# felipefelixarias/a2cat-vn-pytorch

Measured on AMD Instinct MI355X. Metric: env-steps/sec (whole node), 4096 parallel cached-THOR envs at 1/2/4/8 GPUs, higher is better.
Workload: dtype u8; 1 GPU; cached-THOR VectorEnv.step, 20 synthetic 24x24 scenes (626 MB frame cache, HBM-resident), 4096 envs/GPU, 84x84x3 frames, uniform random actions, auto-reset, TimeLimit 900; envs_per_gpu=4096, scenes=20, parallelism=dp1 (independent env shards, replicated scene cache)

## Files before the change

a2cat-vn-pytorch_amd/csrc/vn_env.hip:

```cpp
#include <hip/hip_runtime.h>

#include <algorithm>
#include <cstdlib>
#include <cstring>
#include <mutex>
#include <new>
#include <vector>

#include "vn_common.h"

namespace vn {

static thread_local std::string g_last_error;
void set_error(const std::string& msg) { g_last_error = msg; }
int fail(int code, const std::string& msg) {
  set_error(msg);
  return code;
}
int hip_fail(hipError_t e, const char* what) {
  set_error(std::string(what) + ": " + hipGetErrorString(e));
  return VN_EHIP;
}
const std::string& last_error() { return g_last_error; }

struct SceneDev {
  int64_t row_base;
  int64_t spd_off;
  int64_t cnt_off;
  int64_t comp_base;
  int32_t graph_off;
  int32_t n;
  int32_t maxd;
  int32_t cur_oi;
  int32_t cur_mode;
  float r_goal, r_step, r_coll;
  int32_t terminal_obs;
};

enum { ST_SCENE = 0, ST_STATE, ST_GOAL, ST_OBS, ST_ELAPSED, ST_EPISODE, ST_SCHED, ST_COUNT };

struct EnvArgs {
  const SceneDev* scenes;
  const int32_t* graph;
  const int32_t* spd;
  const uint8_t* arena;
  int64_t frame_bytes;
  int32_t* st;
  float* ep_ret;
  const int32_t* env_scene;
  const int32_t* tasks;
  const int32_t* sched;
  const int32_t* cur_order;
  const int32_t* cur_count;
  uint32_t* flags;
  int n_tasks, sched_len, max_steps, autoreset, n_envs;
  int cur_mode;
  uint32_t k0, k1;
  const int32_t* actions;
  const int32_t* mask;
  uint8_t* obs;
  uint8_t* goal_out;
  float* reward;
  uint8_t* done;
  int32_t* state_out;
  float* info_ret;
  int32_t* info_len;
  int32_t* info_term;
  uint8_t* info_trunc;
  int32_t* info_img_row;
  int32_t* info_goal_row;
  const float* pol_out;
  int pol_A;
  uint32_t pk0, pk1;
  const int64_t* pctr_dev;
  uint64_t pctr;
  int32_t* act_out;
  int64_t* prev_action;
  float* prev_reward;
  float* prev_mask;
  float* lra_next;
  float* mask_next;
  float* stats_env;
  const float* head_w;
  const float* head_b;
  const float* head_x;
  float* head_out;
  uint64_t* rec_addr;
  int32_t* rec_row;
  int reuse;
};

enum { MODE_STEP = 0, MODE_RESET = 1, MODE_OBSERVE = 2, MODE_STEP_HEADS = 3 };
constexpr int kEnvsPerBlock = 4;
constexpr int kStartRounds = 16;

__device__ __forceinline__ int uni(int v) { return __builtin_amdgcn_readfirstlane(v); }

__device__ void reset_env(const EnvArgs& a, int e, int lane, int& sc, int& s, int& g) {
  const int n_envs = a.n_envs;
  const int k = a.st[ST_EPISODE * n_envs + e];
  const int sp = a.st[ST_SCHED * n_envs + e];
  if (a.sched_len > 0 && sp < a.sched_len) {
    sc = a.env_scene[e];
    const int n = a.scenes[sc].n;
    s = a.sched[((int64_t)e * a.sched_len + sp) * 2 + 0];
    g = a.sched[((int64_t)e * a.sched_len + sp) * 2 + 1];
    if ((unsigned)s >= (unsigned)n || (unsigned)g >= (unsigned)n) {
      if (lane == 0) atomicOr(a.flags, (uint32_t)VN_FLAG_BAD_SCHEDULE);
      s = min(max(s, 0), n - 1);
      g = min(max(g, 0), n - 1);
    }
    if (lane == 0) a.st[ST_SCHED * n_envs + e] = sp + 1;
    return;
  }
  const u32x4 rg = philox4x32_10(u32x4{(uint32_t)e, (uint32_t)k, 0u, STREAM_GOAL}, a.k0, a.k1);
  if (a.n_tasks > 0) {
    const int t = (int)uniform_below(rg.x, (uint32_t)a.n_tasks);
    sc = a.tasks[2 * t];
    g = a.tasks[2 * t + 1];
    if (g < 0) g = (int)uniform_below(rg.y, (uint32_t)a.scenes[sc].n);
  } else {
    sc = a.env_scene[e];
    g = (int)uniform_below(rg.x, (uint32_t)a.scenes[sc].n);
  }
  const SceneDev S = a.scenes[sc];
  const int32_t* spd = a.spd + S.spd_off;
  s = -1;
  if (a.cur_mode > 0 && S.cur_mode > 0) {
    const int oi = S.cur_oi;
    const int32_t* cnt = a.cur_count + S.cnt_off + (int64_t)g * (S.maxd + 2);
    const int lo = cnt[1], hi = cnt[oi + 1], n = S.n;
    const u32x4 r = philox4x32_10(u32x4{(uint32_t)e, (uint32_t)k, 0u, STREAM_START}, a.k0, a.k1);
    const bool use_far = (S.cur_mode == 2 && r.y >= 3865470566u && hi < n) || hi <= lo;
    const int b0 = use_far ? hi : lo, b1 = use_far ? n : hi;
    if (b1 > b0) s = a.cur_order[S.spd_off + (int64_t)g * n + b0 + (int)uniform_below(r.x, (uint32_t)(b1 - b0))];
  }
  for (int round = 0; round < kStartRounds && s < 0; ++round) {
    const uint32_t att = (uint32_t)(round * 64 + lane);
    const u32x4 r = philox4x32_10(u32x4{(uint32_t)e, (uint32_t)k, att, STREAM_START}, a.k0, a.k1);
    const int cand = (int)uniform_below(r.x, (uint32_t)S.n);
    const bool ok = spd[(int64_t)cand * S.n + g] > 0;
    const unsigned long long m = __ballot(ok);
    if (m) {
      s = __shfl(cand, __ffsll((long long)m) - 1);
      break;
    }
  }
  if (s < 0) {
    if (lane == 0) atomicOr(a.flags, (uint32_t)VN_FLAG_RESET_EXHAUSTED);
    const u32x4 r = philox4x32_10(u32x4{(uint32_t)e, (uint32_t)k, 0u, STREAM_START}, a.k0, a.k1);
    s = (int)uniform_below(r.x, (uint32_t)S.n);
  }
  s = uni(s);
}

__device__ __forceinline__ void st16_nt(uint4* p, const uint4 v) {
  __builtin_nontemporal_store(v.x, &p->x);
  __builtin_nontemporal_store(v.y, &p->y);
  __builtin_nontemporal_store(v.z, &p->z);
  __builtin_nontemporal_store(v.w, &p->w);
}

template <int VEC>
__device__ __forceinline__ void copy_two_frames(uint8_t* __restrict__ d1, const uint8_t* __restrict__ s1,
                                                uint8_t* __restrict__ d2, const uint8_t* __restrict__ s2,
                                                int64_t bytes, int lane) {
  if constexpr (VEC == 16) {
    constexpr int U = 4;
    const int n = (int)(bytes >> 4);
    const uint4* a = reinterpret_cast<const uint4*>(s1);
    const uint4* b = reinterpret_cast<const uint4*>(s2);
    uint4* x = reinterpret_cast<uint4*>(d1);
    uint4* y = reinterpret_cast<uint4*>(d2);
    int i = lane;
    for (; i + 64 * (U - 1) < n; i += 64 * U) {
      uint4 va[U], vb[U];
#pragma unroll
      for (int u = 0; u < U; ++u) va[u] = a[i + 64 * u];
#pragma unroll
      for (int u = 0; u < U; ++u) vb[u] = b[i + 64 * u];
#pragma unroll
      for (int u = 0; u < U; ++u) st16_nt(x + i + 64 * u, va[u]);
#pragma unroll
      for (int u = 0; u < U; ++u) st16_nt(y + i + 64 * u, vb[u]);
    }
    for (; i < n; i += 64) {
      const uint4 a0 = a[i], b0 = b[i];
      st16_nt(x + i, a0);
      st16_nt(y + i, b0);
    }
  } else if constexpr (VEC == 4) {
    const int n = (int)(bytes >> 2);
    const uint32_t* a = reinterpret_cast<const uint32_t*>(s1);
    const uint32_t* b = reinterpret_cast<const uint32_t*>(s2);
    uint32_t* x = reinterpret_cast<uint32_t*>(d1);
    uint32_t* y = reinterpret_cast<uint32_t*>(d2);
    for (int i = lane; i < n; i += 64) {
      const uint32_t a0 = a[i], b0 = b[i];
      x[i] = a0;
      y[i] = b0;
    }
  } else {
    for (int64_t i = lane; i < bytes; i += 64) {
      d1[i] = s1[i];
      d2[i] = s2[i];
    }
  }
}

template <int VEC>
__device__ __forceinline__ void copy_one_frame(uint8_t* __restrict__ d, const uint8_t* __restrict__ s,
                                               int64_t bytes, int lane) {
  if constexpr (VEC == 16) {
    constexpr int U = 8;
    const int n = (int)(bytes >> 4);
    const uint4* a = reinterpret_cast<const uint4*>(s);
    uint4* x = reinterpret_cast<uint4*>(d);
    int base = 0;
    for (; base + 64 * U <= n; base += 64 * U) {
      const int i = base + lane;
      uint4 v[U];
#pragma unroll
      for (int u = 0; u < U; ++u) v[u] = a[i + 64 * u];
#pragma unroll
      for (int u = 0; u < U; ++u) st16_nt(x + i + 64 * u, v[u]);
    }
    if (base < n) {
      const int i = base + lane;
      uint4 v[U] = {};
#pragma unroll
      for (int u = 0; u < U; ++u)
        if (i + 64 * u < n) v[u] = a[i + 64 * u];
#pragma unroll
      for (int u = 0; u < U; ++u)
        if (i + 64 * u < n) st16_nt(x + i + 64 * u, v[u]);
    }
  } else if constexpr (VEC == 4) {
    const int n = (int)(bytes >> 2);
    const uint32_t* a = reinterpret_cast<const uint32_t*>(s);
    uint32_t* x = reinterpret_cast<uint32_t*>(d);
    for (int i = lane; i < n; i += 64) x[i] = a[i];
  } else {
    for (int64_t i = lane; i < bytes; i += 64) d[i] = s[i];
  }
}

template <int MODE, int VEC>
__global__ __launch_bounds__(256) void env_kernel(EnvArgs a) {
  const int lane = threadIdx.x & 63;
  const int e = uni(blockIdx.x * kEnvsPerBlock + (threadIdx.x >> 6));
  if (e >= a.n_envs) return;
  const int n_envs = a.n_envs;
  int32_t* st = a.st;

  int sc = st[ST_SCENE * n_envs + e];
  int s = st[ST_STATE * n_envs + e];
  int g = st[ST_GOAL * n_envs + e];
  int os = st[ST_OBS * n_envs + e];
  uint64_t rec_a1 = 0, rec_a2 = 0;
  int32_t rec_r1 = -1, rec_r2 = -1;
  if (MODE != MODE_STEP_HEADS && a.reuse) {
    rec_a1 = a.rec_addr[e];
    rec_a2 = a.rec_addr[n_envs + e];
    rec_r1 = a.rec_row[e];
    rec_r2 = a.rec_row[n_envs + e];
  }

  if constexpr (MODE == MODE_STEP || MODE == MODE_STEP_HEADS) {
    int t = st[ST_ELAPSED * n_envs + e];
    const SceneDev S = a.scenes[sc];
    int act;
    if (a.pol_out) {
      float lg[7], p[7], lp[7], H;
      if constexpr (MODE == MODE_STEP_HEADS) {
        const int kl = lane & 31;
        const float* x = a.head_x + (int64_t)e * 512;
        float4 xv[4];
#pragma unroll
        for (int i = 0; i < 4; ++i) xv[i] = *reinterpret_cast<const float4*>(x + 4 * kl + 128 * i);
        float sj[8], bj[8];
#pragma unroll
        for (int j = 0; j < 8; ++j) bj[j] = a.head_b[min(j, a.pol_A)];
#pragma unroll
        for (int j = 0; j < 8; ++j) {
          const float* w = a.head_w + (int64_t)min(j, a.pol_A) * 512;
          float s = 0.0f;
#pragma unroll
          for (int i = 0; i < 4; ++i) {
            const float4 wv = *reinterpret_cast<const float4*>(w + 4 * kl + 128 * i);
            s = fmaf(xv[i].x, wv.x, s);
            s = fmaf(xv[i].y, wv.y, s);
            s = fmaf(xv[i].z, wv.z, s);
            s = fmaf(xv[i].w, wv.w, s);
          }
          sj[j] = s;
        }
#pragma unroll
        for (int j = 0; j < 8; ++j) {
#pragma unroll
          for (int o = 16; o > 0; o >>= 1) sj[j] += __shfl_xor(sj[j], o, 32);
        }
#pragma unroll
        for (int j = 0; j < 8; ++j) {
          if (j <= a.pol_A) {
            const float v = sj[j] + bj[j];
            if (j < a.pol_A) lg[j] = v;
            if (lane == 0) a.head_out[(int64_t)e * 8 + j] = v;
          }
        }
      } else {
        for (int j = 0; j < a.pol_A; ++j) lg[j] = a.pol_out[(int64_t)e * 8 + j];
      }
      const uint64_t ctr = a.pctr + (a.pctr_dev ? (uint64_t)*a.pctr_dev : 0ull);
      act = uni(sample_action(lg, a.pol_A, a.pk0, a.pk1, ctr, (uint32_t)e, p, lp, H));
    } else {
      act = a.actions[e];
    }
    const bool bad = (unsigned)act > 3u;
    int nxt = -1;
    if (!bad) nxt = a.graph[((int64_t)S.graph_off + s) * 4 + act];
    const bool collided = nxt == -1;
    if (!collided) s = nxt;
    const bool terminal = (s == g);
    float r = S.r_step;
    if (terminal) r = S.r_goal;
    if (collided) r = S.r_coll;
    if (!terminal || S.terminal_obs) os = s;
    t += 1;
    const bool limit = a.max_steps > 0 && t >= a.max_steps;
    const bool done = terminal || limit;
    const float ret = a.ep_ret[e] + r;
    const int term_state = os;
    const int ep_len = t;
    float new_ret = ret;
    if (done && a.autoreset) {
      reset_env(a, e, lane, sc, s, g);
      os = s;
      t = 0;
      new_ret = 0.0f;
    }
    if (lane == 0) {
      st[ST_SCENE * n_envs + e] = sc;
      st[ST_STATE * n_envs + e] = s;
      st[ST_GOAL * n_envs + e] = g;
      st[ST_OBS * n_envs + e] = os;
      st[ST_ELAPSED * n_envs + e] = t;
      if (done && a.autoreset) st[ST_EPISODE * n_envs + e] += 1;
      a.ep_ret[e] = new_ret;
      if (bad) atomicOr(a.flags, (uint32_t)VN_FLAG_BAD_ACTION);
      if (a.reward) a.reward[e] = r;
      if (a.done) a.done[e] = done ? 1 : 0;
      if (a.state_out) a.state_out[e] = s;
      if (a.info_ret) a.info_ret[e] = ret;
      if (a.info_len) a.info_len[e] = ep_len;
      if (a.info_term) a.info_term[e] = term_state;
      if (a.info_trunc) a.info_trunc[e] = (limit && !terminal) ? 1 : 0;
      if (a.pol_out) {
        const float m = done ? 0.0f : 1.0f;
        a.act_out[e] = act;
        if (a.prev_action) a.prev_action[e] = act;
        if (a.prev_reward) a.prev_reward[e] = r;
        if (a.prev_mask) a.prev_mask[e] = m;
        if (a.mask_next) a.mask_next[e] = m;
        if (a.lra_next) {
          for (int j = 0; j < a.pol_A; ++j) a.lra_next[(int64_t)e * (a.pol_A + 1) + j] = j == act ? m : 0.0f;
          a.lra_next[(int64_t)e * (a.pol_A + 1) + a.pol_A] = r * m;
        }
        if (a.stats_env && done) {
          a.stats_env[e] += 1.0f;
          a.stats_env[n_envs + e] += ret;
          a.stats_env[2 * (int64_t)n_envs + e] += (float)ep_len;
        }
      }
    }
  } else if constexpr (MODE == MODE_RESET) {
    if (a.mask == nullptr || a.mask[e] != 0) {
      reset_env(a, e, lane, sc, s, g);
      os = s;
      if (lane == 0) {
        st[ST_SCENE * n_envs + e] = sc;
        st[ST_STATE * n_envs + e] = s;
        st[ST_GOAL * n_envs + e] = g;
        st[ST_OBS * n_envs + e] = os;
        st[ST_ELAPSED * n_envs + e] = 0;
        st[ST_EPISODE * n_envs + e] += 1;
        a.ep_ret[e] = 0.0f;
      }
    }
    return;
  } else {
    if (lane == 0 && a.state_out) a.state_out[e] = s;
  }

  const int64_t base = a.scenes[sc].row_base, comp = a.scenes[sc].comp_base;
  const int64_t img_row = base + os, goal_row = comp >= 0 ? comp + os : base + g;
  if (lane == 0) {
    if (a.info_img_row) a.info_img_row[e] = (int32_t)img_row;
    if (a.info_goal_row) a.info_goal_row[e] = (int32_t)goal_row;
  }
  if constexpr (MODE == MODE_STEP_HEADS) return;
  if (a.obs != nullptr && a.goal_out != nullptr) {
    const int64_t F = a.frame_bytes;
    uint8_t* d1 = a.obs + (int64_t)e * F;
    uint8_t* d2 = a.goal_out + (int64_t)e * F;
    const bool keep1 = a.reuse && rec_a1 == (uint64_t)d1 && rec_r1 == (int32_t)img_row;
    const bool keep2 = a.reuse && rec_a2 == (uint64_t)d2 && rec_r2 == (int32_t)goal_row;
    if (!keep1 && !keep2)
      copy_two_frames<VEC>(d1, a.arena + img_row * F, d2, a.arena + goal_row * F, F, lane);
    else if (!keep1)
      copy_one_frame<VEC>(d1, a.arena + img_row * F, F, lane);
    else if (!keep2)
      copy_one_frame<VEC>(d2, a.arena + goal_row * F, F, lane);
    if (lane == 0) {
      a.rec_addr[e] = (uint64_t)d1;
      a.rec_addr[n_envs + e] = (uint64_t)d2;
      a.rec_row[e] = (int32_t)img_row;
      a.rec_row[n_envs + e] = (int32_t)goal_row;
    }
  } else if (a.obs != nullptr || a.goal_out != nullptr) {
    const int64_t F = a.frame_bytes;
    const int k = a.obs ? 0 : 1;
    uint8_t* d = (k == 0 ? a.obs : a.goal_out) + (int64_t)e * F;
    const uint8_t* src = a.arena + (k == 0 ? img_row : goal_row) * F;
    for (int64_t i = lane; i < F; i += 64) d[i] = src[i];
    if (lane == 0) {
      a.rec_addr[k * n_envs + e] = (uint64_t)d;
      a.rec_row[k * n_envs + e] = (int32_t)(k == 0 ? img_row : goal_row);
      if (a.rec_addr[(1 - k) * n_envs + e] == (uint64_t)d) a.rec_addr[(1 - k) * n_envs + e] = 0;
    }
  }
}

__global__ void synth_frames_kernel(uint8_t* arena, int64_t row_base, int n_rows, int64_t frame_bytes,
                                    uint32_t scene_id) {
  const int64_t words = frame_bytes >> 2;
  const int64_t total = words * n_rows;
  uint32_t* dst = reinterpret_cast<uint32_t*>(arena + row_base * frame_bytes);
  for (int64_t i = blockIdx.x * (int64_t)blockDim.x + threadIdx.x; i < total;
       i += (int64_t)gridDim.x * blockDim.x) {
    const int64_t row = i / words, w = i - row * words;
    dst[i] = frame_hash(scene_id, (uint32_t)row, (uint32_t)w);
  }
}

__global__ __launch_bounds__(256) void gather_rows_kernel(const uint8_t* __restrict__ src, int64_t row_bytes,
                                                          const int32_t* __restrict__ rows, int n,
                                                          uint8_t* __restrict__ dst) {
  const int lane = threadIdx.x & 63;
  const int i = uni(blockIdx.x * 4 + (threadIdx.x >> 6));
  if (i >= n) return;
  const uint8_t* s = src + (int64_t)rows[i] * row_bytes;
  uint8_t* d = dst + (int64_t)i * row_bytes;
  if ((row_bytes & 15) == 0) {
    const uint4* a = reinterpret_cast<const uint4*>(s);
    uint4* b = reinterpret_cast<uint4*>(d);
    for (int64_t j = lane; j < (row_bytes >> 4); j += 64) b[j] = a[j];
  } else {
    for (int64_t j = lane; j < row_bytes; j += 64) d[j] = s[j];
  }
}

__global__ void random_actions_kernel(int32_t* actions, int n, uint32_t k0, uint32_t k1, uint64_t step) {
  const int e = blockIdx.x * blockDim.x + threadIdx.x;
  if (e >= n) return;
  const u32x4 r = philox4x32_10(u32x4{(uint32_t)e, (uint32_t)step, (uint32_t)(step >> 32), STREAM_ACTION}, k0, k1);
  actions[e] = (int32_t)(r.x >> 30);
}

}

using namespace vn;

struct vn_ctx {
  int device = 0;
  int n_envs = 0, n_scenes = 0;
  uint64_t seed = 0;
  int64_t frame_bytes = 0, n_rows = 0;
  uint8_t* arena = nullptr;
  int32_t* graph = nullptr;
  int32_t* spd = nullptr;
  SceneDev* scenes = nullptr;
  std::vector<SceneDev> scenes_host;
  int32_t* st = nullptr;
  float* ep_ret = nullptr;
  int32_t* env_scene = nullptr;
  int32_t* tasks = nullptr;
  int n_tasks = 0;
  int32_t* sched = nullptr;
  int sched_len = 0;
  std::vector<int32_t> spd_host;
  int32_t* cur_order = nullptr;
  int32_t* cur_count = nullptr;
  int cur_mode = 0;
  double cur_c = 0.0;
  uint32_t* flags = nullptr;
  int max_steps = 900, autoreset = 1;
  float* info_ret = nullptr;
  int32_t* info_len = nullptr;
  int32_t* info_term = nullptr;
  uint8_t* info_trunc = nullptr;
  int32_t* info_img_row = nullptr;
  int32_t* info_goal_row = nullptr;
  uint64_t* rec_addr = nullptr;
  int32_t* rec_row = nullptr;
  int reuse = 0;
  int reuse_arm = 0;
};

namespace {

struct DeviceGuard {
  int prev = -1;
  explicit DeviceGuard(int d) {
    if (hipGetDevice(&prev) != hipSuccess) prev = -1;
    (void)hipSetDevice(d);
  }
  ~DeviceGuard() {
    if (prev >= 0) (void)hipSetDevice(prev);
  }
};

EnvArgs make_args(vn_ctx* c) {
  EnvArgs a;
  std::memset(&a, 0, sizeof(a));
  a.scenes = c->scenes;
  a.graph = c->graph;
  a.spd = c->spd;
  a.arena = c->arena;
  a.frame_bytes = c->frame_bytes;
  a.st = c->st;
  a.ep_ret = c->ep_ret;
  a.env_scene = c->env_scene;
  a.tasks = c->tasks;
  a.sched = c->sched;
  a.cur_order = c->cur_order;
  a.cur_count = c->cur_count;
  a.cur_mode = c->cur_mode;
  a.flags = c->flags;
  a.n_tasks = c->n_tasks;
  a.sched_len = c->sched_len;
  a.max_steps = c->max_steps;
  a.autoreset = c->autoreset;
  a.n_envs = c->n_envs;
  a.k0 = (uint32_t)c->seed;
  a.k1 = (uint32_t)(c->seed >> 32);
  a.info_ret = c->info_ret;
  a.info_len = c->info_len;
  a.info_term = c->info_term;
  a.info_trunc = c->info_trunc;
  a.info_img_row = c->info_img_row;
  a.info_goal_row = c->info_goal_row;
  a.rec_addr = c->rec_addr;
  a.rec_row = c->rec_row;
  return a;
}

int take_reuse(vn_ctx* c, const uint8_t* obs, const uint8_t* goal, hipStream_t stream) {
  if (!obs || !goal || !c->reuse) return 0;
  if (!c->reuse_arm) return 1;
  hipStreamCaptureStatus cap = hipStreamCaptureStatusNone;
  if (hipStreamIsCapturing(stream, &cap) != hipSuccess) {
    (void)hipGetLastError();
    cap = hipStreamCaptureStatusNone;
  }
  if (cap == hipStreamCaptureStatusNone) c->reuse_arm = 0;
  return 0;
}

template <int MODE>
int launch_env(vn_ctx* c, const EnvArgs& a, hipStream_t stream) {
  const dim3 grid((c->n_envs + kEnvsPerBlock - 1) / kEnvsPerBlock), block(64 * kEnvsPerBlock);
  const int64_t F = c->frame_bytes;
  const bool al16 = (F % 16 == 0) && ((uintptr_t)a.obs % 16 == 0) && ((uintptr_t)a.goal_out % 16 == 0);
  const bool al4 = (F % 4 == 0) && ((uintptr_t)a.obs % 4 == 0) && ((uintptr_t)a.goal_out % 4 == 0);
  if (al16)
    hipLaunchKernelGGL((env_kernel<MODE, 16>), grid, block, 0, stream, a);
  else if (al4)
    hipLaunchKernelGGL((env_kernel<MODE, 4>), grid, block, 0, stream, a);
  else
    hipLaunchKernelGGL((env_kernel<MODE, 1>), grid, block, 0, stream, a);
  VN_HIP(hipGetLastError());
  return VN_OK;
}

void free_ctx(vn_ctx* c) {
  if (!c) return;
  void* ptrs[] = {c->arena, c->graph, c->spd, c->scenes, c->st, c->ep_ret, c->env_scene,
                  c->tasks, c->sched, c->flags, c->cur_order, c->cur_count, c->rec_addr, c->rec_row};
  for (void* p : ptrs)
    if (p) (void)hipFree(p);
  delete c;
}

}

extern "C" {

const char* vn_version(void) { return "vnav 0.1.0 gfx950"; }

int vn_last_error(char* buf, size_t len) {
  if (!buf || len == 0) return VN_EINVAL;
  const std::string& m = vn::last_error();
  const size_t n = std::min(len - 1, m.size());
  std::memcpy(buf, m.data(), n);
  buf[n] = 0;
  return VN_OK;
}

int vn_create(const vn_scene_desc* scenes, int n_scenes, int n_envs, uint64_t seed, int device,
              vn_ctx** out) {
  if (!out) return fail(VN_EINVAL, "vn_create: out is NULL");
  *out = nullptr;
  if (!scenes || n_scenes <= 0) return fail(VN_EINVAL, "vn_create: need at least one scene");
  if (n_envs <= 0) return fail(VN_EINVAL, "vn_create: n_envs must be > 0");
  const int H = scenes[0].height, W = scenes[0].width, C = scenes[0].channels;
  if (H <= 0 || W <= 0 || C <= 0) return fail(VN_EINVAL, "vn_create: bad frame shape");
  const int64_t F = (int64_t)H * W * C;
  int64_t rows = 0, graph_rows = 0, spd_elems = 0;
  std::vector<SceneDev> sh(n_scenes);
  for (int k = 0; k < n_scenes; ++k) {
    const vn_scene_desc& d = scenes[k];
// ... 30 lines not shown
      if (v < -1 || v >= n) return fail(VN_EINVAL, "vn_create: graph entry out of range");
      g32[(int64_t)sh[k].graph_off * 4 + i] = (int32_t)v;
    }
    int32_t mx = 0;
    for (int64_t i = 0; i < n * n; ++i) {
      const int64_t v = d.spd[i];
      spd32[sh[k].spd_off + i] = (int32_t)std::max<int64_t>(std::min<int64_t>(v, INT32_MAX), INT32_MIN);
      mx = std::max(mx, spd32[sh[k].spd_off + i]);
    }
    if (mx > (1 << 20)) return fail(VN_EINVAL, "vn_create: spd values above 2^20");
    sh[k].maxd = mx;
  }
  int64_t cnt_elems = 0;
  for (int k = 0; k < n_scenes; ++k) {
    sh[k].cnt_off = cnt_elems;
    cnt_elems += (int64_t)sh[k].n * (sh[k].maxd + 2);
  }
  DeviceGuard guard(device);
  vn_ctx* c = new (std::nothrow) vn_ctx();
  if (!c) return fail(VN_ENOMEM, "vn_create: host allocation failed");
  c->device = device;
  c->n_envs = n_envs;
  c->n_scenes = n_scenes;
  c->seed = seed;
  c->frame_bytes = F;
  c->n_rows = rows;
  c->scenes_host = sh;
  c->spd_host = spd32;
  auto alloc = [&](void** p, size_t bytes) -> bool {
    return hipMalloc(p, std::max<size_t>(bytes, 16)) == hipSuccess;
  };
  bool ok = alloc((void**)&c->arena, (size_t)(rows * F)) && alloc((void**)&c->graph, g32.size() * 4) &&
            alloc((void**)&c->spd, spd32.size() * 4) && alloc((void**)&c->scenes, sh.size() * sizeof(SceneDev)) &&
            alloc((void**)&c->st, (size_t)ST_COUNT * n_envs * 4) && alloc((void**)&c->ep_ret, (size_t)n_envs * 4) &&
            alloc((void**)&c->env_scene, (size_t)n_envs * 4) && alloc((void**)&c->flags, 4) &&
            alloc((void**)&c->rec_addr, (size_t)2 * n_envs * 8) && alloc((void**)&c->rec_row, (size_t)2 * n_envs * 4);
  if (!ok) {
    free_ctx(c);
    return fail(VN_ENOMEM, "vn_create: device allocation failed");
  }
  hipError_t e = hipSuccess;
  std::vector<int32_t> es(n_envs);
  for (int i = 0; i < n_envs; ++i) es[i] = i % n_scenes;
  if (e == hipSuccess) e = hipMemcpy(c->graph, g32.data(), g32.size() * 4, hipMemcpyHostToDevice);
  if (e == hipSuccess) e = hipMemcpy(c->spd, spd32.data(), spd32.size() * 4, hipMemcpyHostToDevice);
  if (e == hipSuccess) e = hipMemcpy(c->scenes, sh.data(), sh.size() * sizeof(SceneDev), hipMemcpyHostToDevice);
  if (e == hipSuccess) e = hipMemcpy(c->env_scene, es.data(), es.size() * 4, hipMemcpyHostToDevice);
  if (e == hipSuccess) e = hipMemset(c->st, 0, (size_t)ST_COUNT * n_envs * 4);
  if (e == hipSuccess) e = hipMemset(c->ep_ret, 0, (size_t)n_envs * 4);
  if (e == hipSuccess) e = hipMemset(c->flags, 0, 4);
  if (e == hipSuccess) e = hipMemset(c->rec_addr, 0, (size_t)2 * n_envs * 8);
  if (e == hipSuccess) e = hipMemset(c->rec_row, 0, (size_t)2 * n_envs * 4);
  for (int k = 0; k < n_scenes && e == hipSuccess; ++k) {
    const vn_scene_desc& d = scenes[k];
    if (d.companion)
      e = hipMemcpy(c->arena + sh[k].comp_base * F, d.companion, (size_t)d.n_states * F, hipMemcpyHostToDevice);
    if (e != hipSuccess) break;
    if (d.observations) {
      e = hipMemcpy(c->arena + sh[k].row_base * F, d.observations, (size_t)d.n_states * F, hipMemcpyHostToDevice);
    } else {
      hipLaunchKernelGGL(synth_frames_kernel, dim3(2048), dim3(256), 0, 0, c->arena, sh[k].row_base, d.n_states, F,
                         d.synth_id);
      e = hipGetLastError();
    }
  }
  if (e != hipSuccess) {
    free_ctx(c);
    return hip_fail(e, "vn_create: upload");
  }
  EnvArgs a = make_args(c);
  int rc = launch_env<MODE_RESET>(c, a, 0);
  if (rc == VN_OK) {
    e = hipDeviceSynchronize();
    if (e != hipSuccess) rc = hip_fail(e, "vn_create: initial reset");
  }
  if (rc != VN_OK) {
    free_ctx(c);
    return rc;
  }
  *out = c;
  return VN_OK;
}

int vn_destroy(vn_ctx* c) {
  if (!c) return VN_OK;
// ... 75 lines not shown
    return launch_env<MODE_STEP_HEADS>(c, a, (hipStream_t)stream);
  }
  return launch_env<MODE_STEP>(c, a, (hipStream_t)stream);
}

int vn_set_info_buffers(vn_ctx* c, float* ep_return, int32_t* ep_length, int32_t* terminal_state,
                        uint8_t* truncated, int32_t* img_row, int32_t* goal_row) {
  if (!c) return fail(VN_EINVAL, "vn_set_info_buffers: NULL ctx");
  c->info_ret = ep_return;
  c->info_len = ep_length;
  c->info_term = terminal_state;
  c->info_trunc = truncated;
  c->info_img_row = img_row;
  c->info_goal_row = goal_row;
  return VN_OK;
}

int vn_set_schedule(vn_ctx* c, const int32_t* start_goal_dev, int len) {
  if (!c) return fail(VN_EINVAL, "vn_set_schedule: NULL ctx");
  if (len < 0 || (len > 0 && !start_goal_dev)) return fail(VN_EINVAL, "vn_set_schedule: bad schedule");
  DeviceGuard guard(c->device);
  if (c->sched) {
    VN_HIP(hipDeviceSynchronize());
    VN_HIP(hipFree(c->sched));
    c->sched = nullptr;
  }
  c->sched_len = 0;
  if (len > 0) {
    const size_t bytes = (size_t)c->n_envs * len * 2 * 4;
    if (hipMalloc((void**)&c->sched, bytes) != hipSuccess) return fail(VN_ENOMEM, "vn_set_schedule: alloc");
    VN_HIP(hipMemcpy(c->sched, start_goal_dev, bytes, hipMemcpyDefault));
    c->sched_len = len;
  }
  VN_HIP(hipMemset(c->st + (size_t)ST_SCHED * c->n_envs, 0, (size_t)c->n_envs * 4));
  return VN_OK;
}

int vn_set_tasks(vn_ctx* c, const int32_t* tasks_host, int n_tasks) {
  if (!c) return fail(VN_EINVAL, "vn_set_tasks: NULL ctx");
  if (n_tasks < 0 || (n_tasks > 0 && !tasks_host)) return fail(VN_EINVAL, "vn_set_tasks: bad tasks");
  for (int t = 0; t < n_tasks; ++t) {
    const int sc = tasks_host[2 * t], g = tasks_host[2 * t + 1];
    if (sc < 0 || sc >= c->n_scenes) return fail(VN_EINVAL, "vn_set_tasks: scene out of range");
    if (g < -1 || g >= c->scenes_host[sc].n) return fail(VN_EINVAL, "vn_set_tasks: goal out of range");
  }
  DeviceGuard guard(c->device);
  if (c->tasks) {
    VN_HIP(hipDeviceSynchronize());
    VN_HIP(hipFree(c->tasks));
    c->tasks = nullptr;
  }
  c->n_tasks = 0;
  if (n_tasks > 0) {
    if (hipMalloc((void**)&c->tasks, (size_t)n_tasks * 8) != hipSuccess) return fail(VN_ENOMEM, "vn_set_tasks: alloc");
    VN_HIP(hipMemcpy(c->tasks, tasks_host, (size_t)n_tasks * 8, hipMemcpyHostToDevice));
    c->n_tasks = n_tasks;
  }
  return VN_OK;
}

int vn_set_env_scenes(vn_ctx* c, const int32_t* env_scene_host) {
  if (!c || !env_scene_host) return fail(VN_EINVAL, "vn_set_env_scenes: NULL argument");
  for (int e = 0; e < c->n_envs; ++e)
    if (env_scene_host[e] < 0 || env_scene_host[e] >= c->n_scenes)
      return fail(VN_EINVAL, "vn_set_env_scenes: scene out of range");
  DeviceGuard guard(c->device);
  VN_HIP(hipMemcpy(c->env_scene, env_scene_host, (size_t)c->n_envs * 4, hipMemcpyHostToDevice));
// ... 72 lines not shown
  c->autoreset = on ? 1 : 0;
  return VN_OK;
}

int vn_set_output_reuse(vn_ctx* c, int on) {
  if (!c) return fail(VN_EINVAL, "vn_set_output_reuse: NULL ctx");
  c->reuse = on ? 1 : 0;
  c->reuse_arm = c->reuse;
  return VN_OK;
}

int vn_random_actions(vn_ctx* c, int32_t* actions_dev, uint64_t step, vn_stream_t stream) {
  if (!c || !actions_dev) return fail(VN_EINVAL, "vn_random_actions: NULL argument");
  DeviceGuard guard(c->device);
  hipLaunchKernelGGL(random_actions_kernel, dim3((c->n_envs + 255) / 256), dim3(256), 0, (hipStream_t)stream,
                     actions_dev, c->n_envs, (uint32_t)c->seed ^ 0xA5A5A5A5u, (uint32_t)(c->seed >> 32), step);
  VN_HIP(hipGetLastError());
  return VN_OK;
}

int vn_gather_rows(const uint8_t* src_dev, int64_t row_bytes, const int32_t* rows_dev, int n, uint8_t* dst_dev,
                   vn_stream_t stream) {
  if (!src_dev || !rows_dev || !dst_dev || row_bytes <= 0 || n < 0) return fail(VN_EINVAL, "vn_gather_rows: bad args");
  if (n == 0) return VN_OK;
  hipLaunchKernelGGL(gather_rows_kernel, dim3((n + 3) / 4), dim3(256), 0, (hipStream_t)stream, src_dev, row_bytes,
                     rows_dev, n, dst_dev);
  VN_HIP(hipGetLastError());
  return VN_OK;
}

int vn_get_state(vn_ctx* c, int32_t* dst, vn_stream_t stream) {
  if (!c || !dst) return fail(VN_EINVAL, "vn_get_state: NULL argument");
  DeviceGuard guard(c->device);
  VN_HIP(hipMemcpyAsync(dst, c->st, (size_t)ST_COUNT * c->n_envs * 4, hipMemcpyDeviceToDevice, (hipStream_t)stream));
  return VN_OK;
}

int vn_set_state(vn_ctx* c, const int32_t* src, vn_stream_t stream) {
  if (!c || !src) return fail(VN_EINVAL, "vn_set_state: NULL argument");
  DeviceGuard guard(c->device);
  VN_HIP(hipMemcpyAsync(c->st, src, (size_t)ST_COUNT * c->n_envs * 4, hipMemcpyDeviceToDevice, (hipStream_t)stream));
  return VN_OK;
}

int vn_get_episode_returns(vn_ctx* c, float* dst, vn_stream_t stream) {
  if (!c || !dst) return fail(VN_EINVAL, "vn_get_episode_returns: NULL argument");
  DeviceGuard guard(c->device);
  VN_HIP(hipMemcpyAsync(dst, c->ep_ret, (size_t)c->n_envs * 4, hipMemcpyDeviceToDevice, (hipStream_t)stream));
  return VN_OK;
}

int vn_set_episode_returns(vn_ctx* c, const float* src, vn_stream_t stream) {
  if (!c || !src) return fail(VN_EINVAL, "vn_set_episode_returns: NULL argument");
  DeviceGuard guard(c->device);
  VN_HIP(hipMemcpyAsync(c->ep_ret, src, (size_t)c->n_envs * 4, hipMemcpyDeviceToDevice, (hipStream_t)stream));
  return VN_OK;
}

int vn_frame_arena(vn_ctx* c, const uint8_t** arena, int64_t* frame_bytes, int64_t* n_rows) {
  if (!c) return fail(VN_EINVAL, "vn_frame_arena: NULL ctx");
  if (arena) *arena = c->arena;
  if (frame_bytes) *frame_bytes = c->frame_bytes;
  if (n_rows) *n_rows = c->n_rows;
  return VN_OK;
}

int vn_scene_row_base(vn_ctx* c, int scene, int64_t* row_base) {
  if (!c || !row_base || scene < 0 || scene >= c->n_scenes) return fail(VN_EINVAL, "vn_scene_row_base: bad args");
  *row_base = c->scenes_host[scene].row_base;
  return VN_OK;
}

int vn_error_flags_sync(vn_ctx* c, uint32_t* flags, int clear) {
  if (!c || !flags) return fail(VN_EINVAL, "vn_error_flags_sync: NULL argument");
  DeviceGuard guard(c->device);
  VN_HIP(hipDeviceSynchronize());
  VN_HIP(hipMemcpy(flags, c->flags, 4, hipMemcpyDeviceToHost));
  if (clear) VN_HIP(hipMemset(c->flags, 0, 4));
  return VN_OK;
}

}
```

Baseline: 136.3 million env-steps/s.

## Pack per-env state into 128-byte records with cached neighbors and scene data

```diff
diff --git a/a2cat-vn-pytorch_amd/csrc/vn_env.hip b/a2cat-vn-pytorch_amd/csrc/vn_env.hip
--- a/a2cat-vn-pytorch_amd/csrc/vn_env.hip
+++ b/a2cat-vn-pytorch_amd/csrc/vn_env.hip
@@ -39,14 +39,38 @@
 
 enum { ST_SCENE = 0, ST_STATE, ST_GOAL, ST_OBS, ST_ELAPSED, ST_EPISODE, ST_SCHED, ST_COUNT };
 
+enum {
+  RW_ST = 0,
+  RW_RET = 7,
+  RW_NB = 8,
+  RW_ROW_BASE = 12,
+  RW_COMP_BASE = 13,
+  RW_GRAPH_TOBS = 14,
+  RW_R_GOAL = 15,
+  RW_R_STEP = 16,
+  RW_R_COLL = 17,
+  RW_OUT_ROW = 18,
+  RW_OUT_ADDR = 20,
+  RW_USED = 24,
+  RW_WORDS = 32,
+};
+struct alignas(128) EnvRec {
+  int32_t w[RW_WORDS];
+};
+static_assert(sizeof(EnvRec) == 128, "one record per 128-B line");
+
+typedef int32_t i32x16 __attribute__((ext_vector_type(16), may_alias, aligned(64)));
+typedef int32_t i32x8 __attribute__((ext_vector_type(8), may_alias, aligned(32)));
+typedef int32_t i32x4 __attribute__((ext_vector_type(4), may_alias, aligned(16)));
+typedef int32_t i32x2 __attribute__((ext_vector_type(2), may_alias, aligned(8)));
+
 struct EnvArgs {
   const SceneDev* scenes;
   const int32_t* graph;
   const int32_t* spd;
   const uint8_t* arena;
   int64_t frame_bytes;
-  int32_t* st;
-  float* ep_ret;
+  EnvRec* recs;
   const int32_t* env_scene;
   const int32_t* tasks;
   const int32_t* sched;
@@ -85,8 +109,6 @@
   const float* head_b;
   const float* head_x;
   float* head_out;
-  uint64_t* rec_addr;
-  int32_t* rec_row;
   int reuse;
 };
 
@@ -96,10 +118,7 @@
 
 __device__ __forceinline__ int uni(int v) { return __builtin_amdgcn_readfirstlane(v); }
 
-__device__ void reset_env(const EnvArgs& a, int e, int lane, int& sc, int& s, int& g) {
-  const int n_envs = a.n_envs;
-  const int k = a.st[ST_EPISODE * n_envs + e];
-  const int sp = a.st[ST_SCHED * n_envs + e];
+__device__ void reset_env(const EnvArgs& a, int e, int lane, int k, int& sp, int& sc, int& s, int& g) {
   if (a.sched_len > 0 && sp < a.sched_len) {
     sc = a.env_scene[e];
     const int n = a.scenes[sc].n;
@@ -110,7 +129,7 @@
       s = min(max(s, 0), n - 1);
       g = min(max(g, 0), n - 1);
     }
-    if (lane == 0) a.st[ST_SCHED * n_envs + e] = sp + 1;
+    sp += 1;
     return;
   }
   const u32x4 rg = philox4x32_10(u32x4{(uint32_t)e, (uint32_t)k, 0u, STREAM_GOAL}, a.k0, a.k1);
@@ -161,10 +180,10 @@
   __builtin_nontemporal_store(v.w, &p->w);
 }
 
-template <int VEC>
+template <int VEC, class Mid>
 __device__ __forceinline__ void copy_two_frames(uint8_t* __restrict__ d1, const uint8_t* __restrict__ s1,
                                                 uint8_t* __restrict__ d2, const uint8_t* __restrict__ s2,
-                                                int64_t bytes, int lane) {
+                                                int64_t bytes, int lane, Mid mid) {
   if constexpr (VEC == 16) {
     constexpr int U = 4;
     const int n = (int)(bytes >> 4);
@@ -173,6 +192,23 @@
     uint4* x = reinterpret_cast<uint4*>(d1);
     uint4* y = reinterpret_cast<uint4*>(d2);
     int i = lane;
+    {
+      const bool full = 64 * U <= n;
+      const int i0 = full ? lane : min(lane, n - 1), step = full ? 64 : 0;
+      uint4 va[U], vb[U];
+#pragma unroll
+      for (int u = 0; u < U; ++u) va[u] = a[i0 + step * u];
+#pragma unroll
+      for (int u = 0; u < U; ++u) vb[u] = b[i0 + step * u];
+      mid();
+      if (full) {
+#pragma unroll
+        for (int u = 0; u < U; ++u) st16_nt(x + i + 64 * u, va[u]);
+#pragma unroll
+        for (int u = 0; u < U; ++u) st16_nt(y + i + 64 * u, vb[u]);
+        i += 64 * U;
+      }
+    }
     for (; i + 64 * (U - 1) < n; i += 64 * U) {
       uint4 va[U], vb[U];
 #pragma unroll
@@ -190,6 +226,7 @@
       st16_nt(y + i, b0);
     }
   } else if constexpr (VEC == 4) {
+    mid();
     const int n = (int)(bytes >> 2);
     const uint32_t* a = reinterpret_cast<const uint32_t*>(s1);
     const uint32_t* b = reinterpret_cast<const uint32_t*>(s2);
@@ -201,6 +238,7 @@
       y[i] = b0;
     }
   } else {
+    mid();
     for (int64_t i = lane; i < bytes; i += 64) {
       d1[i] = s1[i];
       d2[i] = s2[i];
@@ -208,15 +246,28 @@
   }
 }
 
-template <int VEC>
+template <int VEC, class Mid>
 __device__ __forceinline__ void copy_one_frame(uint8_t* __restrict__ d, const uint8_t* __restrict__ s,
-                                               int64_t bytes, int lane) {
+                                               int64_t bytes, int lane, Mid mid) {
   if constexpr (VEC == 16) {
     constexpr int U = 8;
     const int n = (int)(bytes >> 4);
     const uint4* a = reinterpret_cast<const uint4*>(s);
     uint4* x = reinterpret_cast<uint4*>(d);
     int base = 0;
+    {
+      const bool full = 64 * U <= n;
+      const int i0 = full ? lane : min(lane, n - 1), step = full ? 64 : 0;
+      uint4 v[U];
+#pragma unroll
+      for (int u = 0; u < U; ++u) v[u] = a[i0 + step * u];
+      mid();
+      if (full) {
+#pragma unroll
+        for (int u = 0; u < U; ++u) st16_nt(x + lane + 64 * u, v[u]);
+        base = 64 * U;
+      }
+    }
     for (; base + 64 * U <= n; base += 64 * U) {
       const int i = base + lane;
       uint4 v[U];
@@ -236,13 +287,35 @@
         if (i + 64 * u < n) st16_nt(x + i + 64 * u, v[u]);
     }
   } else if constexpr (VEC == 4) {
+    mid();
     const int n = (int)(bytes >> 2);
     const uint32_t* a = reinterpret_cast<const uint32_t*>(s);
     uint32_t* x = reinterpret_cast<uint32_t*>(d);
     for (int i = lane; i < n; i += 64) x[i] = a[i];
   } else {
+    mid();
     for (int64_t i = lane; i < bytes; i += 64) d[i] = s[i];
   }
+}
+
+struct SceneCache {
+  int32_t row_base, comp_base;
+  uint32_t graph_tobs;
+  float r_goal, r_step, r_coll;
+};
+__device__ __forceinline__ SceneCache scene_cache(const SceneDev& S) {
+  return SceneCache{(int32_t)S.row_base, (int32_t)S.comp_base,
+                    ((uint32_t)S.graph_off << 1) | (S.terminal_obs != 0 ? 1u : 0u), S.r_goal, S.r_step, S.r_coll};
+}
+__device__ __forceinline__ void store_scene_cache(EnvRec* R, const SceneCache& c) {
+  *reinterpret_cast<i32x4*>(R->w + RW_ROW_BASE) =
+      i32x4{c.row_base, c.comp_base, (int32_t)c.graph_tobs, __float_as_int(c.r_goal)};
+  *reinterpret_cast<i32x2*>(R->w + RW_R_STEP) = i32x2{__float_as_int(c.r_step), __float_as_int(c.r_coll)};
+}
+__device__ __forceinline__ void store_out_record(EnvRec* R, int32_t row1, int32_t row2, uint64_t a1, uint64_t a2) {
+  *reinterpret_cast<i32x2*>(R->w + RW_OUT_ROW) = i32x2{row1, row2};
+  *reinterpret_cast<i32x4*>(R->w + RW_OUT_ADDR) =
+      i32x4{(int32_t)(uint32_t)a1, (int32_t)(uint32_t)(a1 >> 32), (int32_t)(uint32_t)a2, (int32_t)(uint32_t)(a2 >> 32)};
 }
 
 template <int MODE, int VEC>
@@ -251,25 +324,28 @@
   const int e = uni(blockIdx.x * kEnvsPerBlock + (threadIdx.x >> 6));
   if (e >= a.n_envs) return;
   const int n_envs = a.n_envs;
-  int32_t* st = a.st;
-
-  int sc = st[ST_SCENE * n_envs + e];
-  int s = st[ST_STATE * n_envs + e];
-  int g = st[ST_GOAL * n_envs + e];
-  int os = st[ST_OBS * n_envs + e];
-  uint64_t rec_a1 = 0, rec_a2 = 0;
-  int32_t rec_r1 = -1, rec_r2 = -1;
-  if (MODE != MODE_STEP_HEADS && a.reuse) {
-    rec_a1 = a.rec_addr[e];
-    rec_a2 = a.rec_addr[n_envs + e];
-    rec_r1 = a.rec_row[e];
-    rec_r2 = a.rec_row[n_envs + e];
-  }
+  EnvRec* R = a.recs + e;
+
+  const i32x16 lo = *reinterpret_cast<const i32x16*>(R->w);
+  const i32x8 hi = *reinterpret_cast<const i32x8*>(R->w + 16);
+  int sc = lo[ST_SCENE], s = lo[ST_STATE], g = lo[ST_GOAL], os = lo[ST_OBS];
+  int t = lo[ST_ELAPSED], ep = lo[ST_EPISODE], sp = lo[ST_SCHED];
+  SceneCache C{lo[RW_ROW_BASE], lo[RW_COMP_BASE], (uint32_t)lo[RW_GRAPH_TOBS], __int_as_float(lo[RW_R_GOAL]),
+               __int_as_float(hi[RW_R_STEP - 16]), __int_as_float(hi[RW_R_COLL - 16])};
+  const int32_t rec_r1 = hi[RW_OUT_ROW - 16], rec_r2 = hi[RW_OUT_ROW + 1 - 16];
+  const uint64_t rec_a1 = (uint32_t)hi[RW_OUT_ADDR - 16] | ((uint64_t)(uint32_t)hi[RW_OUT_ADDR + 1 - 16] << 32);
+  const uint64_t rec_a2 = (uint32_t)hi[RW_OUT_ADDR + 2 - 16] | ((uint64_t)(uint32_t)hi[RW_OUT_ADDR + 3 - 16] << 32);
+
+  int act_in = 0;
+  if constexpr (MODE == MODE_STEP) {
+    if (a.actions) act_in = a.actions[e];
+  }
+
+  bool scene_changed = false, bad = false, done = false, limit = false, terminal = false;
+  int act = 0, term_state = 0, ep_len = 0;
+  float r = 0.0f, ret = 0.0f, new_ret = 0.0f;
 
   if constexpr (MODE == MODE_STEP || MODE == MODE_STEP_HEADS) {
-    int t = st[ST_ELAPSED * n_envs + e];
-    const SceneDev S = a.scenes[sc];
-    int act;
     if (a.pol_out) {
       float lg[7], p[7], lp[7], H;
       if constexpr (MODE == MODE_STEP_HEADS) {
@@ -314,39 +390,66 @@
       const uint64_t ctr = a.pctr + (a.pctr_dev ? (uint64_t)*a.pctr_dev : 0ull);
       act = uni(sample_action(lg, a.pol_A, a.pk0, a.pk1, ctr, (uint32_t)e, p, lp, H));
     } else {
-      act = a.actions[e];
-    }
-    const bool bad = (unsigned)act > 3u;
+      act = act_in;
+    }
+    bad = (unsigned)act > 3u;
     int nxt = -1;
-    if (!bad) nxt = a.graph[((int64_t)S.graph_off + s) * 4 + act];
+    if (!bad) nxt = act == 0 ? lo[RW_NB] : act == 1 ? lo[RW_NB + 1] : act == 2 ? lo[RW_NB + 2] : lo[RW_NB + 3];
     const bool collided = nxt == -1;
     if (!collided) s = nxt;
-    const bool terminal = (s == g);
-    float r = S.r_step;
-    if (terminal) r = S.r_goal;
-    if (collided) r = S.r_coll;
-    if (!terminal || S.terminal_obs) os = s;
+    terminal = (s == g);
+    r = C.r_step;
+    if (terminal) r = C.r_goal;
+    if (collided) r = C.r_coll;
+    if (!terminal || (C.graph_tobs & 1u)) os = s;
     t += 1;
-    const bool limit = a.max_steps > 0 && t >= a.max_steps;
-    const bool done = terminal || limit;
-    const float ret = a.ep_ret[e] + r;
-    const int term_state = os;
-    const int ep_len = t;
-    float new_ret = ret;
+    limit = a.max_steps > 0 && t >= a.max_steps;
+    done = terminal || limit;
+    ret = __int_as_float(lo[RW_RET]) + r;
+    term_state = os;
+    ep_len = t;
+    new_ret = ret;
     if (done && a.autoreset) {
-      reset_env(a, e, lane, sc, s, g);
+      reset_env(a, e, lane, ep, sp, sc, s, g);
       os = s;
       t = 0;
+      ep += 1;
       new_ret = 0.0f;
-    }
-    if (lane == 0) {
-      st[ST_SCENE * n_envs + e] = sc;
-      st[ST_STATE * n_envs + e] = s;
-      st[ST_GOAL * n_envs + e] = g;
-      st[ST_OBS * n_envs + e] = os;
-      st[ST_ELAPSED * n_envs + e] = t;
-      if (done && a.autoreset) st[ST_EPISODE * n_envs + e] += 1;
-      a.ep_ret[e] = new_ret;
+      C = scene_cache(a.scenes[sc]);
+      scene_changed = true;
+    }
+  } else if constexpr (MODE == MODE_RESET) {
+    if (a.mask == nullptr || a.mask[e] != 0) {
+      reset_env(a, e, lane, ep, sp, sc, s, g);
+      C = scene_cache(a.scenes[sc]);
+      const i32x4 nb = *reinterpret_cast<const i32x4*>(a.graph + ((int64_t)(C.graph_tobs >> 1) + s) * 4);
+      if (lane == 0) {
+        *reinterpret_cast<i32x4*>(R->w + 0) = i32x4{sc, s, g, s};
+        *reinterpret_cast<i32x4*>(R->w + 4) = i32x4{0, ep + 1, sp, __float_as_int(0.0f)};
+        *reinterpret_cast<i32x4*>(R->w + RW_NB) = nb;
+        store_scene_cache(R, C);
+      }
+    }
+    return;
+  }
+
+  i32x4 nb = i32x4{lo[RW_NB], lo[RW_NB + 1], lo[RW_NB + 2], lo[RW_NB + 3]};
+  if constexpr (MODE == MODE_STEP || MODE == MODE_STEP_HEADS)
+    nb = *reinterpret_cast<const i32x4*>(a.graph + ((int64_t)(C.graph_tobs >> 1) + s) * 4);
+
+  const int32_t img_row = C.row_base + os, goal_row = C.comp_base >= 0 ? C.comp_base + os : C.row_base + g;
+
+  auto emit = [&](bool out_rec, int32_t row1, int32_t row2, uint64_t addr1, uint64_t addr2)
+                  __attribute__((always_inline)) {
+    if (lane != 0) return;
+    if constexpr (MODE == MODE_STEP || MODE == MODE_STEP_HEADS) {
+      *reinterpret_cast<i32x4*>(R->w + 0) = i32x4{sc, s, g, os};
+      *reinterpret_cast<i32x4*>(R->w + 4) = i32x4{t, ep, sp, __float_as_int(new_ret)};
+      *reinterpret_cast<i32x4*>(R->w + RW_NB) = nb;
+      if (scene_changed) store_scene_cache(R, C);
+    }
+    if (out_rec) store_out_record(R, row1, row2, addr1, addr2);
+    if constexpr (MODE == MODE_STEP || MODE == MODE_STEP_HEADS) {
       if (bad) atomicOr(a.flags, (uint32_t)VN_FLAG_BAD_ACTION);
       if (a.reward) a.reward[e] = r;
       if (a.done) a.done[e] = done ? 1 : 0;
@@ -355,6 +458,12 @@
       if (a.info_len) a.info_len[e] = ep_len;
       if (a.info_term) a.info_term[e] = term_state;
       if (a.info_trunc) a.info_trunc[e] = (limit && !terminal) ? 1 : 0;
+    } else {
+      if (a.state_out) a.state_out[e] = s;
+    }
+    if (a.info_img_row) a.info_img_row[e] = img_row;
+    if (a.info_goal_row) a.info_goal_row[e] = goal_row;
+    if constexpr (MODE == MODE_STEP || MODE == MODE_STEP_HEADS) {
       if (a.pol_out) {
         const float m = done ? 0.0f : 1.0f;
         a.act_out[e] = act;
@@ -373,62 +482,67 @@
         }
       }
     }
-  } else if constexpr (MODE == MODE_RESET) {
-    if (a.mask == nullptr || a.mask[e] != 0) {
-      reset_env(a, e, lane, sc, s, g);
-      os = s;
-      if (lane == 0) {
-        st[ST_SCENE * n_envs + e] = sc;
-        st[ST_STATE * n_envs + e] = s;
-        st[ST_GOAL * n_envs + e] = g;
-        st[ST_OBS * n_envs + e] = os;
-        st[ST_ELAPSED * n_envs + e] = 0;
-        st[ST_EPISODE * n_envs + e] += 1;
-        a.ep_ret[e] = 0.0f;
-      }
-    }
+  };
+
+  if constexpr (MODE == MODE_STEP_HEADS) {
+    emit(false, 0, 0, 0, 0);
     return;
-  } else {
-    if (lane == 0 && a.state_out) a.state_out[e] = s;
-  }
-
-  const int64_t base = a.scenes[sc].row_base, comp = a.scenes[sc].comp_base;
-  const int64_t img_row = base + os, goal_row = comp >= 0 ? comp + os : base + g;
-  if (lane == 0) {
-    if (a.info_img_row) a.info_img_row[e] = (int32_t)img_row;
-    if (a.info_goal_row) a.info_goal_row[e] = (int32_t)goal_row;
-  }
-  if constexpr (MODE == MODE_STEP_HEADS) return;
+  }
   if (a.obs != nullptr && a.goal_out != nullptr) {
     const int64_t F = a.frame_bytes;
     uint8_t* d1 = a.obs + (int64_t)e * F;
     uint8_t* d2 = a.goal_out + (int64_t)e * F;
-    const bool keep1 = a.reuse && rec_a1 == (uint64_t)d1 && rec_r1 == (int32_t)img_row;
-    const bool keep2 = a.reuse && rec_a2 == (uint64_t)d2 && rec_r2 == (int32_t)goal_row;
-    if (!keep1 && !keep2)
-      copy_two_frames<VEC>(d1, a.arena + img_row * F, d2, a.arena + goal_row * F, F, lane);
-    else if (!keep1)
-      copy_one_frame<VEC>(d1, a.arena + img_row * F, F, lane);
-    else if (!keep2)
-      copy_one_frame<VEC>(d2, a.arena + goal_row * F, F, lane);
-    if (lane == 0) {
-      a.rec_addr[e] = (uint64_t)d1;
-      a.rec_addr[n_envs + e] = (uint64_t)d2;
-      a.rec_row[e] = (int32_t)img_row;
-      a.rec_row[n_envs + e] = (int32_t)goal_row;
+    const bool keep1 = a.reuse && rec_a1 == (uint64_t)d1 && rec_r1 == img_row;
+    const bool keep2 = a.reuse && rec_a2 == (uint64_t)d2 && rec_r2 == goal_row;
+    auto mid = [&]() __attribute__((always_inline)) { emit(true, img_row, goal_row, (uint64_t)d1, (uint64_t)d2); };
+    if (!keep1 && !keep2) {
+      copy_two_frames<VEC>(d1, a.arena + (int64_t)img_row * F, d2, a.arena + (int64_t)goal_row * F, F, lane, mid);
+    } else if (!keep1 || !keep2) {
+      uint8_t* d = keep1 ? d2 : d1;
+      const int32_t row = keep1 ? goal_row : img_row;
+      copy_one_frame<VEC>(d, a.arena + (int64_t)row * F, F, lane, mid);
+    } else {
+      mid();
     }
   } else if (a.obs != nullptr || a.goal_out != nullptr) {
     const int64_t F = a.frame_bytes;
     const int k = a.obs ? 0 : 1;
     uint8_t* d = (k == 0 ? a.obs : a.goal_out) + (int64_t)e * F;
-    const uint8_t* src = a.arena + (k == 0 ? img_row : goal_row) * F;
+    const uint8_t* src = a.arena + (int64_t)(k == 0 ? img_row : goal_row) * F;
+    const uint64_t oa = k == 0 ? rec_a2 : rec_a1;
+    const uint64_t other = oa == (uint64_t)d ? 0 : oa;
+    if (k == 0)
+      emit(true, img_row, rec_r2, (uint64_t)d, other);
+    else
+      emit(true, rec_r1, goal_row, other, (uint64_t)d);
     for (int64_t i = lane; i < F; i += 64) d[i] = src[i];
-    if (lane == 0) {
-      a.rec_addr[k * n_envs + e] = (uint64_t)d;
-      a.rec_row[k * n_envs + e] = (int32_t)(k == 0 ? img_row : goal_row);
-      if (a.rec_addr[(1 - k) * n_envs + e] == (uint64_t)d) a.rec_addr[(1 - k) * n_envs + e] = 0;
-    }
-  }
+  } else {
+    emit(false, 0, 0, 0, 0);
+  }
+}
+
+__global__ void rec_gather_kernel(const EnvRec* recs, int n_envs, int w0, int nw, int32_t* dst) {
+  const int e = blockIdx.x * blockDim.x + threadIdx.x;
+  if (e >= n_envs) return;
+  for (int f = 0; f < nw; ++f) dst[(int64_t)f * n_envs + e] = recs[e].w[w0 + f];
+}
+
+__global__ void rec_scatter_kernel(EnvRec* recs, int n_envs, int w, const int32_t* src) {
+  const int e = blockIdx.x * blockDim.x + threadIdx.x;
+  if (e >= n_envs) return;
+  recs[e].w[w] = src ? src[e] : 0;
+}
+
+__global__ void set_state_kernel(EnvRec* recs, int n_envs, const int32_t* src, const SceneDev* scenes,
+                                 int n_scenes, const int32_t* graph) {
+  const int e = blockIdx.x * blockDim.x + threadIdx.x;
+  if (e >= n_envs) return;
+  EnvRec* R = recs + e;
+  for (int f = 0; f < ST_COUNT; ++f) R->w[RW_ST + f] = src[(int64_t)f * n_envs + e];
+  const SceneDev S = scenes[min(max(src[(int64_t)ST_SCENE * n_envs + e], 0), n_scenes - 1)];
+  const int s = min(max(src[(int64_t)ST_STATE * n_envs + e], 0), S.n - 1);
+  *reinterpret_cast<i32x4*>(R->w + RW_NB) = *reinterpret_cast<const i32x4*>(graph + ((int64_t)S.graph_off + s) * 4);
+  store_scene_cache(R, scene_cache(S));
 }
 
 __global__ void synth_frames_kernel(uint8_t* arena, int64_t row_base, int n_rows, int64_t frame_bytes,
@@ -481,8 +595,7 @@
   int32_t* spd = nullptr;
   SceneDev* scenes = nullptr;
   std::vector<SceneDev> scenes_host;
-  int32_t* st = nullptr;
-  float* ep_ret = nullptr;
+  EnvRec* recs = nullptr;
   int32_t* env_scene = nullptr;
   int32_t* tasks = nullptr;
   int n_tasks = 0;
@@ -501,8 +614,6 @@
   uint8_t* info_trunc = nullptr;
   int32_t* info_img_row = nullptr;
   int32_t* info_goal_row = nullptr;
-  uint64_t* rec_addr = nullptr;
-  int32_t* rec_row = nullptr;
   int reuse = 0;
   int reuse_arm = 0;
 };
@@ -528,8 +639,7 @@
   a.spd = c->spd;
   a.arena = c->arena;
   a.frame_bytes = c->frame_bytes;
-  a.st = c->st;
-  a.ep_ret = c->ep_ret;
+  a.recs = c->recs;
   a.env_scene = c->env_scene;
   a.tasks = c->tasks;
   a.sched = c->sched;
@@ -550,8 +660,6 @@
   a.info_trunc = c->info_trunc;
   a.info_img_row = c->info_img_row;
   a.info_goal_row = c->info_goal_row;
-  a.rec_addr = c->rec_addr;
-  a.rec_row = c->rec_row;
   return a;
 }
 
@@ -585,8 +693,8 @@
 
 void free_ctx(vn_ctx* c) {
   if (!c) return;
-  void* ptrs[] = {c->arena, c->graph, c->spd, c->scenes, c->st, c->ep_ret, c->env_scene,
-                  c->tasks, c->sched, c->flags, c->cur_order, c->cur_count, c->rec_addr, c->rec_row};
+  void* ptrs[] = {c->arena, c->graph, c->spd, c->scenes, c->recs, c->env_scene,
+                  c->tasks, c->sched, c->flags, c->cur_order, c->cur_count};
   for (void* p : ptrs)
     if (p) (void)hipFree(p);
   delete c;
@@ -683,9 +791,8 @@
   };
   bool ok = alloc((void**)&c->arena, (size_t)(rows * F)) && alloc((void**)&c->graph, g32.size() * 4) &&
             alloc((void**)&c->spd, spd32.size() * 4) && alloc((void**)&c->scenes, sh.size() * sizeof(SceneDev)) &&
-            alloc((void**)&c->st, (size_t)ST_COUNT * n_envs * 4) && alloc((void**)&c->ep_ret, (size_t)n_envs * 4) &&
-            alloc((void**)&c->env_scene, (size_t)n_envs * 4) && alloc((void**)&c->flags, 4) &&
-            alloc((void**)&c->rec_addr, (size_t)2 * n_envs * 8) && alloc((void**)&c->rec_row, (size_t)2 * n_envs * 4);
+            alloc((void**)&c->recs, (size_t)n_envs * sizeof(EnvRec)) &&
+            alloc((void**)&c->env_scene, (size_t)n_envs * 4) && alloc((void**)&c->flags, 4);
   if (!ok) {
     free_ctx(c);
     return fail(VN_ENOMEM, "vn_create: device allocation failed");
@@ -697,11 +804,8 @@
   if (e == hipSuccess) e = hipMemcpy(c->spd, spd32.data(), spd32.size() * 4, hipMemcpyHostToDevice);
   if (e == hipSuccess) e = hipMemcpy(c->scenes, sh.data(), sh.size() * sizeof(SceneDev), hipMemcpyHostToDevice);
   if (e == hipSuccess) e = hipMemcpy(c->env_scene, es.data(), es.size() * 4, hipMemcpyHostToDevice);
-  if (e == hipSuccess) e = hipMemset(c->st, 0, (size_t)ST_COUNT * n_envs * 4);
-  if (e == hipSuccess) e = hipMemset(c->ep_ret, 0, (size_t)n_envs * 4);
+  if (e == hipSuccess) e = hipMemset(c->recs, 0, (size_t)n_envs * sizeof(EnvRec));
   if (e == hipSuccess) e = hipMemset(c->flags, 0, 4);
-  if (e == hipSuccess) e = hipMemset(c->rec_addr, 0, (size_t)2 * n_envs * 8);
-  if (e == hipSuccess) e = hipMemset(c->rec_row, 0, (size_t)2 * n_envs * 4);
   for (int k = 0; k < n_scenes && e == hipSuccess; ++k) {
     const vn_scene_desc& d = scenes[k];
     if (d.companion)
@@ -843,7 +947,9 @@
     VN_HIP(hipMemcpy(c->sched, start_goal_dev, bytes, hipMemcpyDefault));
     c->sched_len = len;
   }
-  VN_HIP(hipMemset(c->st + (size_t)ST_SCHED * c->n_envs, 0, (size_t)c->n_envs * 4));
+  hipLaunchKernelGGL(rec_scatter_kernel, dim3((c->n_envs + 255) / 256), dim3(256), 0, 0, c->recs, c->n_envs,
+                     RW_ST + ST_SCHED, (const int32_t*)nullptr);
+  VN_HIP(hipGetLastError());
   return VN_OK;
 }
 
@@ -982,28 +1088,36 @@
 int vn_get_state(vn_ctx* c, int32_t* dst, vn_stream_t stream) {
   if (!c || !dst) return fail(VN_EINVAL, "vn_get_state: NULL argument");
   DeviceGuard guard(c->device);
-  VN_HIP(hipMemcpyAsync(dst, c->st, (size_t)ST_COUNT * c->n_envs * 4, hipMemcpyDeviceToDevice, (hipStream_t)stream));
+  hipLaunchKernelGGL(rec_gather_kernel, dim3((c->n_envs + 255) / 256), dim3(256), 0, (hipStream_t)stream, c->recs,
+                     c->n_envs, RW_ST, ST_COUNT, dst);
+  VN_HIP(hipGetLastError());
   return VN_OK;
 }
 
 int vn_set_state(vn_ctx* c, const int32_t* src, vn_stream_t stream) {
   if (!c || !src) return fail(VN_EINVAL, "vn_set_state: NULL argument");
   DeviceGuard guard(c->device);
-  VN_HIP(hipMemcpyAsync(c->st, src, (size_t)ST_COUNT * c->n_envs * 4, hipMemcpyDeviceToDevice, (hipStream_t)stream));
+  hipLaunchKernelGGL(set_state_kernel, dim3((c->n_envs + 255) / 256), dim3(256), 0, (hipStream_t)stream, c->recs,
+                     c->n_envs, src, c->scenes, c->n_scenes, c->graph);
+  VN_HIP(hipGetLastError());
   return VN_OK;
 }
 
 int vn_get_episode_returns(vn_ctx* c, float* dst, vn_stream_t stream) {
   if (!c || !dst) return fail(VN_EINVAL, "vn_get_episode_returns: NULL argument");
   DeviceGuard guard(c->device);
-  VN_HIP(hipMemcpyAsync(dst, c->ep_ret, (size_t)c->n_envs * 4, hipMemcpyDeviceToDevice, (hipStream_t)stream));
+  hipLaunchKernelGGL(rec_gather_kernel, dim3((c->n_envs + 255) / 256), dim3(256), 0, (hipStream_t)stream, c->recs,
+                     c->n_envs, RW_RET, 1, reinterpret_cast<int32_t*>(dst));
+  VN_HIP(hipGetLastError());
   return VN_OK;
 }
 
 int vn_set_episode_returns(vn_ctx* c, const float* src, vn_stream_t stream) {
   if (!c || !src) return fail(VN_EINVAL, "vn_set_episode_returns: NULL argument");
   DeviceGuard guard(c->device);
-  VN_HIP(hipMemcpyAsync(c->ep_ret, src, (size_t)c->n_envs * 4, hipMemcpyDeviceToDevice, (hipStream_t)stream));
+  hipLaunchKernelGGL(rec_scatter_kernel, dim3((c->n_envs + 255) / 256), dim3(256), 0, (hipStream_t)stream, c->recs,
+                     c->n_envs, RW_RET, reinterpret_cast<const int32_t*>(src));
+  VN_HIP(hipGetLastError());
   return VN_OK;
 }
 
```

After: 145.2 million env-steps/s, median of 6. 6.5% higher.
